# qucontrol/krotov

Hardware: AMD Instinct MI355X
Metric: state*timestep propagations/s (Krotov iterations/s in iterations_per_sec), 256-objective N=64 ensemble (higher is better)
Workload: dtype f64

## Files before the change

krotov_amd/csrc/kh_common.h:

```cpp
#pragma once

#include <hip/hip_runtime.h>
#include <stdint.h>

typedef double2 cplx;

#define KH_TU_ALL 0
#define KH_TU_MAIN 1
#define KH_TU_GENERIC 2
#define KH_TU_MINI 3
#define KH_TU_TILE 4
#define KH_TU_Q2 5
#define KH_TU_STREAM 6
#define KH_TU_ENS 7
#define KH_TU_TILEN 8
#define KH_TU_COOP_STORE 9
#define KH_TU_COOP_UPDATE_A 10
#define KH_TU_COOP_UPDATE_B 11
#define KH_TU_ELL_STORE 12
#define KH_TU_ELL_UPDATE_A 13
#define KH_TU_ELL_UPDATE_B 14
#define KH_TU_TILEX 15
#define KH_TU_LIND 16
#ifndef KH_TU
// ... 70 lines not shown
    int lo = __builtin_amdgcn_readfirstlane(__double2loint(v));
    int hi = __builtin_amdgcn_readfirstlane(__double2hiint(v));
    return __hiloint2double(hi, lo);
}

__device__ __forceinline__ double sum64(double v) {
    v = sum16(v);
    return (readlane_f64(v, 0) + readlane_f64(v, 16)) + (readlane_f64(v, 32) + readlane_f64(v, 48));
}

__device__ __forceinline__ double sum64_mfma(double v) {
    double d = __builtin_amdgcn_mfma_f64_4x4x4f64(v, 1.0, 0.0, 0, 0, 0);
    d += dpp_move<KH_DPP_ROR8>(d);
    d += dpp_move<KH_DPP_ROR4>(d);
    return __builtin_amdgcn_mfma_f64_4x4x4f64(d, 1.0, 0.0, 0, 0, 0);
}

__host__ inline void kh_build_degree_table(double tol, double *tab ) {
    tab[0] = 0.0;
    for (int m = 1; m <= KH_MAX_DEGREE; ++m) {
        double lo = 0.0, hi = (double)(m + 2) * (1.0 - 1e-12);
        for (int it = 0; it < 200; ++it) {
            const double th = 0.5 * (lo + hi);
            double term = 1.0;
            for (int j = 1; j <= m + 1; ++j) term *= th / j;
            if (term <= tol * (1.0 - th / (m + 2))) lo = th; else hi = th;
        }
        tab[m] = lo;
    }
}

#define KH_Q2_ROWS (KH_MAX_DEGREE / 2)

#define KH_RATIO_STRIDE (KH_MAX_DEGREE + 1)

__host__ inline void kh_build_taylor_rows(double *c0 , double *rows ,
                                          double *ratios ) {
    for (int m = 0; m <= KH_MAX_DEGREE; ++m) {
        c0[m] = 1.0;
        ratios[(size_t)m * KH_RATIO_STRIDE] = 1.0;
        for (int j = 1; j <= KH_MAX_DEGREE; ++j) ratios[(size_t)m * KH_RATIO_STRIDE + j] = 1.0 / j;
        for (int p = 0; p < KH_Q2_ROWS; ++p) {
            rows[((size_t)m * KH_Q2_ROWS + p) * 2 + 0] = 1.0 / (2 * p + 1);
            rows[((size_t)m * KH_Q2_ROWS + p) * 2 + 1] = 1.0 / ((2.0 * p + 1) * (2 * p + 2));
        }
    }
}

__host__ inline void kh_bessel_j(double theta, int kmax, long double *J) {
    const int start = kmax + 40 + (int)(2.0 * theta);
    long double jp = 0.0L, jc = 1e-300L, norm = 0.0L;
    for (int k = start; k >= 1; --k) {
        const long double jm = (2.0L * k / (long double)theta) * jc - jp;
        jp = jc;
        jc = jm;
        if (k - 1 <= kmax) J[k - 1] = jc;
        if (((k - 1) & 1) == 0) norm += (k - 1 == 0 ? 1.0L : 2.0L) * jc;
        if (fabsl(jc) > 1e200L) {
            jc *= 1e-200L;
            jp *= 1e-200L;
            norm *= 1e-200L;
            for (int q = k - 1; q <= kmax; ++q) J[q] *= 1e-200L;
        }
    }
    for (int k = 0; k <= kmax; ++k) J[k] /= norm;
}

__host__ inline long double kh_bernstein_eta(long double d) {
    const long double a = sqrtl(fmaxl(0.0L, 1.0L - d * d));
    const long double xr = -2.0L * d * d, xi = 2.0L * a * d;
    const long double r = sqrtl(xr * xr + xi * xi);
    const long double sr = sqrtl(fmaxl(0.0L, 0.5L * (r + xr))), si = sqrtl(fmaxl(0.0L, 0.5L * (r - xr)));
    const long double p = hypotl(a + sr, d + si), q = hypotl(a - sr, d - si);
    return logl(p > q ? p : q);
}
__host__ inline void kh_build_real_spectrum_rows(double tol, double *tab , double *c0, double *rows,
                                                 double *ratios, double theta_cap = 2.0, double delta = 0.0) {
    const int TAIL = 40;
    long double J[KH_MAX_DEGREE + TAIL + 2];
    auto err = [&](double theta, int m) {
        kh_bessel_j(theta, m + TAIL, J);
        long double e = 0.0L;
        if (delta > 0.0) {
            const long double d = (long double)delta / (long double)theta;
            const long double eta = d < 1.0L ? kh_bernstein_eta(d) : 1e3L;
            for (int k = m + 1; k <= m + TAIL; ++k) e += fabsl(J[k]) * coshl(k * eta);
            return (double)(2.0L * (1.0L + sqrtl(2.0L)) * e);
        }
        for (int k = m + 1; k <= m + TAIL; ++k) e += fabsl(J[k]);
        return (double)(2.0L * e);
    };
    kh_build_taylor_rows(c0, rows, ratios);
    double taylor_tab[KH_MAX_DEGREE + 1];
    kh_build_degree_table(tol, taylor_tab);
    tab[0] = 0.0;
    for (int m = 1; m <= KH_MAX_DEGREE; ++m) {
        if (m & 1) {
            tab[m] = tab[m - 1];
            continue;
        }
        if (taylor_tab[m] >= theta_cap) {
            tab[m] = taylor_tab[m] > tab[m - 1] ? taylor_tab[m] : tab[m - 1];
            continue;
        }
        double lo = 0.0, hi = theta_cap;
        if (err(hi, m) <= tol) {
            lo = hi;
        } else {
            for (int it = 0; it < 60; ++it) {
                const double th = 0.5 * (lo + hi);
                if (err(th, m) <= tol) lo = th; else hi = th;
            }
        }
        if (lo < tab[m - 1]) lo = tab[m - 1];
        tab[m] = lo;
        const double theta = lo;
        if (!(theta > 0.0)) continue;
        static long double T[KH_MAX_DEGREE + 1][KH_MAX_DEGREE + 1];
        for (int k = 0; k <= m; ++k)
            for (int j = 0; j <= m; ++j) T[k][j] = 0.0L;
        T[0][0] = 1.0L;
        if (m >= 1) T[1][1] = 1.0L;
        for (int k = 1; k < m; ++k)
            for (int j = 0; j <= k + 1; ++j) T[k + 1][j] = (j > 0 ? 2.0L * T[k][j - 1] : 0.0L) - T[k - 1][j];
        kh_bessel_j(theta, m, J);
        long double c[KH_MAX_DEGREE + 1];
        for (int j = 0; j <= m; ++j) {
            long double acc = 0.0L;
            for (int k = j; k <= m; k += 2)
                acc += (k == 0 ? 1.0L : 2.0L) * J[k] * T[k][j] * (((k - j) / 2) % 2 ? -1.0L : 1.0L);
            c[j] = acc / powl((long double)theta, j);
        }
        c0[m] = (double)c[0];
        ratios[(size_t)m * KH_RATIO_STRIDE] = (double)c[0];
        for (int j = 1; j <= m; ++j) ratios[(size_t)m * KH_RATIO_STRIDE + j] = (double)(j == 1 ? c[1] : c[j] / c[j - 1]);
        for (int p = 0; 2 * p + 2 <= m && p < KH_Q2_ROWS; ++p) {
            const long double den = p == 0 ? 1.0L : c[2 * p];
            rows[((size_t)m * KH_Q2_ROWS + p) * 2 + 0] = (double)(c[2 * p + 1] / den);
            rows[((size_t)m * KH_Q2_ROWS + p) * 2 + 1] = (double)(c[2 * p + 2] / den);
        }
    }
}

struct KhDegreeCache {
    int m;
    double lo, hi;
};

__device__ __forceinline__ void kh_degree_cached(double theta, const double *tab, double theta_max,
                                                 double inv_theta_max, KhDegreeCache &c, int *s_out, int *m_out) {
    int s = 1;
    double th = theta;
    if (theta > theta_max) {
        s = (int)ceil(theta * inv_theta_max);
        th = theta / s;
    }
    if (!(th > c.lo && th <= c.hi)) {
        int m = c.m < 1 ? 1 : c.m;
        while (m > 1 && th <= tab[m - 1]) --m;
        while (m < KH_MAX_DEGREE && th > tab[m]) ++m;
        c.m = m;
        c.lo = m > 1 ? tab[m - 1] : -1.0;
        c.hi = m < KH_MAX_DEGREE ? tab[m] : 1e300;
    }
    *s_out = s;
    *m_out = c.m;
}

__device__ __forceinline__ void kh_degree_lookup(double theta, const double *__restrict__ tab, double theta_max,
                                                 double inv_theta_max, int hint, int *s_out, int *m_out) {
    int s = 1;
    double th = theta;
// ... 262 lines not shown
```

krotov_amd/csrc/kh_coop.h:

```cpp
#pragma once

#include "kh_common.h"
#include "kh_generic.h"

#define KH_COOP_THREADS 512
#define KH_COOP_WAVES 8
#define KH_COOP_COLS 16
#define KH_COOP_RING 32
#ifndef KH_COOP_RING_LOCAL
#define KH_COOP_RING_LOCAL 4
#endif
#ifndef KH_COOP_CHUNK
#define KH_COOP_CHUNK 4
#endif
#define KH_COOP_MAX_L 2

typedef double kh_d4 __attribute__((ext_vector_type(4)));

template <int COLS>
__device__ __forceinline__ bool kh_coop_is_owner(int tid) {
    if constexpr (COLS == 2) return (tid & 15) == 0;
    return tid < 16 * COLS;
}
template <int COLS>
// ... 819 lines not shown
                state.y += t.y;
                if (owner_valid) kh_coop_publish<COLS>(c, rid + 1, y, row, col, j == m ? state : t, c.local != 0);
            }
            ++rid;
        }
    }
    return true;
}

#define KH_COOP_REFRESH 64
struct KhCoopSqMasks {
    unsigned int h0, h1, p0, p1, p2;
};
__device__ __forceinline__ KhCoopSqMasks kh_coop_sq_masks(const KhCoopArgs &c, int g, int wave) {
    KhCoopSqMasks m = {0u, 0u, 0u, 0u, 0u};
    if (c.sq != nullptr) {
        m.h0 = kh_coop_frag_mask(c.tab[0], c.G, g, wave, c.ks);
        m.h1 = kh_coop_frag_mask(c.tab[1], c.G, g, wave, c.ks);
        m.p0 = kh_coop_frag_mask(c.tab[2], c.G, g, wave, c.ks);
        m.p1 = kh_coop_frag_mask(c.tab[3], c.G, g, wave, c.ks);
        m.p2 = kh_coop_frag_mask(c.tab[4], c.G, g, wave, c.ks);
    }
    return m;
}
template <int MAXKS>
__device__ __forceinline__ void kh_coop_sq_restart(const KhCoopArgs &c, const KhCoopSqMasks &mk, int g, int wave,
                                                   int lane, const KhCoopFrag &a, cplx (&breg)[MAXKS],
                                                   double &eps_prev) {
    kh_coop_reg_load<MAXKS>(c.tab[2], g, wave, lane, c.ks, breg, mk.p0);
    kh_coop_load_frag<MAXKS>(c.tab[0], g, wave, lane, c.ks, a, mk.h0);
    eps_prev = 0.0;
}

template <int MAXKS, int COLS>
__device__ __forceinline__ bool kh_coop_expm_action_sq(const KhCoopArgs &c, const KhExchange &ex,
                                                       const KhCoopSqMasks &mk, double eps, double &eps_prev, const KhCoopFrag &a,
                                                       cplx (&breg)[MAXKS],
                                                       cplx &state, unsigned int &rid, KhCoopLds &s, int N, int y,
                                                       int g, int row, int col, bool owner_valid, double fre,
                                                       double fim, double dt, int nsub, int m, int tid, int wave,
                                                       int lane, const cplx (*p1pre)[MAXKS] = nullptr) {
    const double h = kh_uniform(nsub == 1 ? dt : dt / nsub);
    const double f2h2 = kh_uniform((fre * fre - fim * fim) * h * h);
    const int phases = (m + 1) >> 1;
    const bool series = c.ser_rows != nullptr;
    if (series) {
        const double *grow = c.ser_rows + (size_t)m * KH_Q2_ROWS * 2;
        if (tid < 2 * phases) s.coef[tid] = grow[tid];
        if (tid == 2 * phases) s.coef[tid] = c.ser_c0[m];
        __syncthreads();
    }
    const double *rows = series ? s.coef : nullptr;
    const double c_0 = kh_uniform(series ? s.coef[2 * phases] : 1.0), c_1 = kh_uniform(series ? s.coef[0] : 1.0);
#ifndef KH_COOP_X_NOREBUILD
    {
#ifdef KH_TIMING
        const long long tr0 = clock64();
#endif
        const double e1 = eps - eps_prev, e2 = e1 * (eps + eps_prev);
        if (p1pre != nullptr) {
            kh_coop_axpy_pair<MAXKS>(c.tab[4], e2, breg, c.tab[1], e1, a, g, wave, lane, c.ks, mk.p2 | mk.h1);
#pragma unroll
            for (int q = 0; q < MAXKS; ++q) {
                breg[q].x = fma(e1, (*p1pre)[q].x, breg[q].x);
                breg[q].y = fma(e1, (*p1pre)[q].y, breg[q].y);
            }
        } else {
            kh_coop_reg_axpy<MAXKS>(c.tab[3], e1, g, wave, lane, c.ks, breg, mk.p1);
            kh_coop_reg_axpy<MAXKS>(c.tab[4], e2, g, wave, lane, c.ks, breg, mk.p2);
            kh_coop_axpy_frag<MAXKS>(c.tab[1], e1, g, wave, lane, c.ks, a, mk.h1);
        }
        eps_prev = kh_uniform(eps);
#ifdef KH_TIMING
        if (tid == 0 && blockIdx.x == 0) {
            const long long tr1 = clock64();
            s.tim[10] += (double)(tr1 - tr0);
            if (s.tim[11] != 0.0) s.tim[11] += (double)(tr1 - tr0);
        }
#endif
    }
#endif
    const KhCoopRegFrag<MAXKS> bf = {breg, ~0u};
    for (int sub = 0; sub < nsub; ++sub) {
        cplx sacc = c_make(h * c_1 * state.x, h * c_1 * state.y);
        state = c_make(c_0 * state.x, c_0 * state.y);
        for (int ph = 0; ph < phases; ++ph) {
            const double r2 = rows != nullptr ? rows[2 * ph + 1] : kh_inv_table[2 * ph + 1] * kh_inv_table[2 * ph + 2];
            const double r1n = ph + 1 < phases ? (rows != nullptr ? rows[2 * ph + 2] : kh_inv_table[2 * ph + 3]) : 0.0;
            cplx w;
            kh_coop_round<MAXKS, COLS>(c, ex, rid, y, N, bf, s, tid, wave, lane, w);
            const double c2 = f2h2 * r2, hn = h * r1n;
            if (kh_coop_is_owner<COLS>(tid)) {
                const cplx t2 = c_make(c2 * w.x, c2 * w.y);
                state.x += t2.x;
                state.y += t2.y;
                const bool last = (ph + 1 == phases);
                if (!last) {
                    sacc.x = fma(hn, t2.x, sacc.x);
                    sacc.y = fma(hn, t2.y, sacc.y);
                }
                if (owner_valid) kh_coop_publish<COLS>(c, rid + 1, y, row, col, last ? sacc : t2, c.local != 0);
            }
            ++rid;
        }
        cplx w;
        kh_coop_round<MAXKS, COLS>(c, ex, rid, y, N, a, s, tid, wave, lane, w);
        if (s.abort) return false;
        if (kh_coop_is_owner<COLS>(tid)) {
            const cplx odd = c_mul(c_make(fre, fim), w);
            state.x += odd.x;
            state.y += odd.y;
            if (owner_valid) kh_coop_publish<COLS>(c, rid + 1, y, row, col, state, c.local != 0);
        }
        ++rid;
    }
    return true;
}

template <int MAXKS, int COLS>
__device__ __forceinline__ bool kh_coop_expm_action_sq_ahead(const KhCoopArgs &c, const KhExchange &ex, const KhCoopSqMasks &mk,
                                                             double eps, double eps_next, bool have_next, double &eps_b,
                                                             double &eps_a, const KhCoopFrag &a, cplx (&breg)[MAXKS],
                                                             cplx &state, unsigned int &rid, KhCoopLds &s, int N, int y, int g,
                                                             int row, int col, bool owner_valid, double fre, double fim,
                                                             double dt, int nsub, int m, int tid, int wave, int lane) {
    static_assert(MAXKS % 4 == 0, "quarters");
    const double h = kh_uniform(nsub == 1 ? dt : dt / nsub);
    const double f2h2 = kh_uniform((fre * fre - fim * fim) * h * h);
    const int phases = (m + 1) >> 1;
    const bool series = c.ser_rows != nullptr;
    if (series) {
        const double *grow = c.ser_rows + (size_t)m * KH_Q2_ROWS * 2;
        if (tid < 2 * phases) s.coef[tid] = grow[tid];
        if (tid == 2 * phases) s.coef[tid] = c.ser_c0[m];
        __syncthreads();
    }
    const double *rows = series ? s.coef : nullptr;
    const double c_0 = kh_uniform(series ? s.coef[2 * phases] : 1.0), c_1 = kh_uniform(series ? s.coef[0] : 1.0);
    if (eps_b != eps) {
        const double e1 = eps - eps_b, e2 = e1 * (eps + eps_b);
        kh_coop_reg_axpy<MAXKS>(c.tab[3], e1, g, wave, lane, c.ks, breg, mk.p1);
        kh_coop_reg_axpy<MAXKS>(c.tab[4], e2, g, wave, lane, c.ks, breg, mk.p2);
        eps_b = kh_uniform(eps);
    }
    const auto advance_a = [&]() {
        if (eps_a != eps) {
            kh_coop_axpy_frag<MAXKS>(c.tab[1], eps - eps_a, g, wave, lane, c.ks, a, mk.h1);
            eps_a = kh_uniform(eps);
        }
    };
    const KhCoopRegFrag<MAXKS> bf = {breg, ~0u};
    const KhCoopSrc src1 = kh_coop_frag_src(c.tab[3], g, wave, lane, c.ks);
    constexpr int QS = MAXKS / 4;
    for (int sub = 0; sub < nsub; ++sub) {
        const bool ahead = have_next && sub + 1 == nsub;
        const bool staged = ahead && phases >= 4;
        cplx p1n[MAXKS];
#pragma unroll
        for (int q = 0; q < MAXKS; ++q) p1n[q] = c_make(0.0, 0.0);
        cplx sacc = c_make(h * c_1 * state.x, h * c_1 * state.y);
        state = c_make(c_0 * state.x, c_0 * state.y);
        const auto b_round = [&](int ph, const auto &hook2) {
            const double r2 = rows != nullptr ? rows[2 * ph + 1] : kh_inv_table[2 * ph + 1] * kh_inv_table[2 * ph + 2];
            const double r1n = ph + 1 < phases ? (rows != nullptr ? rows[2 * ph + 2] : kh_inv_table[2 * ph + 3]) : 0.0;
            cplx w;
            kh_coop_round<MAXKS, COLS>(c, ex, rid, y, N, bf, s, tid, wave, lane, w, advance_a, hook2);
            const double c2 = f2h2 * r2, hn = h * r1n;
            if (kh_coop_is_owner<COLS>(tid)) {
                const cplx t2 = c_make(c2 * w.x, c2 * w.y);
                state.x += t2.x;
                state.y += t2.y;
                const bool last = (ph + 1 == phases);
                if (!last) {
                    sacc.x = fma(hn, t2.x, sacc.x);
                    sacc.y = fma(hn, t2.y, sacc.y);
                }
                if (owner_valid) kh_coop_publish<COLS>(c, rid + 1, y, row, col, last ? sacc : t2, c.local != 0);
            }
            ++rid;
        };
        const int plain_rounds = staged ? phases - 4 : phases;
        for (int ph = 0; ph < plain_rounds; ++ph) b_round(ph, KhNoHook());
        if (staged) {
            b_round(phases - 4, [&]() {
#pragma unroll
                for (int j = 0; j < QS; ++j) p1n[0 * QS + j] = src1[(size_t)(0 * QS + j) * 64];
            });
            b_round(phases - 3, [&]() {
#pragma unroll
                for (int j = 0; j < QS; ++j) p1n[1 * QS + j] = src1[(size_t)(1 * QS + j) * 64];
            });
            b_round(phases - 2, [&]() {
#pragma unroll
                for (int j = 0; j < QS; ++j) p1n[2 * QS + j] = src1[(size_t)(2 * QS + j) * 64];
            });
            b_round(phases - 1, [&]() {
#pragma unroll
                for (int j = 0; j < QS; ++j) p1n[3 * QS + j] = src1[(size_t)(3 * QS + j) * 64];
            });
        }
        advance_a();
        if (ahead && !staged) kh_coop_reg_load<MAXKS>(c.tab[3], g, wave, lane, c.ks, p1n, mk.p1);
        const auto advance_b = [&]() {
            if (ahead) {
                const double e1 = eps_next - eps_b, e2 = e1 * (eps_next + eps_b);
#pragma unroll
                for (int q = 0; q < MAXKS; ++q) {
                    breg[q].x = fma(e1, p1n[q].x, breg[q].x);
                    breg[q].y = fma(e1, p1n[q].y, breg[q].y);
                }
                kh_coop_reg_axpy<MAXKS>(c.tab[4], e2, g, wave, lane, c.ks, breg, mk.p2);
                eps_b = kh_uniform(eps_next);
            }
        };
        cplx w;
        kh_coop_round<MAXKS, COLS>(c, ex, rid, y, N, a, s, tid, wave, lane, w, advance_b);
        if (s.abort) return false;
        if (kh_coop_is_owner<COLS>(tid)) {
            const cplx odd = c_mul(c_make(fre, fim), w);
            state.x += odd.x;
            state.y += odd.y;
            if (owner_valid) kh_coop_publish<COLS>(c, rid + 1, y, row, col, state, c.local != 0);
        }
        ++rid;
    }
    return true;
}

__global__ void kh_coop_adj_mask_kernel(const cplx *__restrict__ op , int N, int G,
// ... 93 lines not shown
    const KhCoopFrag a = {(cplx *)s.frag + tid};
    cplx breg[MAXKS];
    double eps_prev = 0.0, eps_a = 0.0;
    const KhCoopSqMasks mk = kh_coop_sq_masks(c, g, wave);
#pragma unroll
    for (int q = 0; q < MAXKS; ++q) breg[q] = c_make(0.0, 0.0);
    for (int step = 0; step < nt - 1; ++step) {
        const int n = direction > 0 ? step : nt - 2 - step;
        if (SQ && step % KH_COOP_REFRESH == 0) {
            kh_coop_sq_restart<MAXKS>(c, mk, g, wave, lane, a, breg, eps_prev);
            eps_a = 0.0;
        }
        double eps[KH_COOP_MAX_L];
        double theta = p.op_norms[0];
#pragma unroll
        for (int l = 0; l < KH_COOP_MAX_L; ++l) {
            eps[l] = 0.0;
            if (l < L) {
                eps[l] = pulses[(size_t)l * (nt - 1) + n];
                theta += fabs(eps[l]) * p.op_norms[1 + l];
            }
        }
        const double dt = p.dt[n];
        int nsub, m;
        kh_degree_lookup(theta * dt, s.deg, p.theta_max, p.inv_theta_max, m_hint, &nsub, &m);
        m_hint = m;
        if constexpr (SQ) {
            const bool have_next = step + 1 < nt - 1;
            const double eps_next = have_next ? pulses[direction > 0 ? n + 1 : n - 1] : 0.0;
            if (!kh_coop_expm_action_sq_ahead<MAXKS, COLS>(c, ex, mk, eps[0], eps_next, have_next, eps_prev, eps_a, a, breg, state,
                                                           rid, s, N, y, g, row, col, owner_valid, p.fre, p.fim, dt, nsub, m, tid,
                                                           wave, lane))
                return;
            rounds += (double)nsub * (((m + 1) >> 1) + 1);
        } else {
            kh_coop_build<MAXKS>(c.fops, eps, L, g, wave, lane, c.ks, a);
            if (!kh_coop_expm_action<MAXKS, COLS>(c, ex, a, state, rid, s, N, y, row, col, owner_valid, p.fre, p.fim, dt,
                                                  nsub, m, tid, wave, lane))
                return;
            rounds += (double)nsub * m;
        }
        if (has_state && store != nullptr) store[((size_t)k * nt + (direction > 0 ? n + 1 : n)) * N + row] = state;
    }
    if (has_state && state_out != nullptr) state_out[(size_t)k * N + row] = state;
    if (g == 0 && tid == 0 && p.stats != nullptr) {
        const int cols = min(c.cols, p.K - y * c.cols);
        atomicAdd(p.stats, rounds * cols);
#ifdef KH_TIMING
        if (y == 0) {
            p.stats[1] = s.tim[0] / rounds + 1e6 * (double)(long long)(s.tim[4] / rounds);
            p.stats[2] = s.tim[1] / rounds + 1e6 * (double)(long long)(100.0 * s.tim[5] / rounds);
            p.stats[3] = s.tim[2] / rounds + 1e6 * (double)(long long)(100.0 * s.tim[6] / rounds);
            p.stats[4] = 0.0;
            p.stats[5] = s.tim[0] / rounds;
            p.stats[6] = p.stats[5] + s.tim[1] / rounds;
            p.stats[7] = p.stats[6] + s.tim[2] / rounds;
            p.stats[8] = p.stats[7] + s.tim[7] / rounds;
            p.stats[9] = p.stats[8] + s.tim[8] / rounds;
            p.stats[10] = p.stats[9] + s.tim[9] / rounds;
            p.stats[11] = s.tim[10] / (nt - 1);
            p.stats[12] = 1.0 + s.local;
            p.stats[13] = 0.0;
        }
#endif
    }
}

// ... 125 lines not shown
            }
#ifdef KH_TIMING
            if (g == 0 && lane == 0 && p.stats != nullptr && y < 16) p.stats[20 + y] += (double)(clock64() - tx0) / (nt - 1);
#endif
#endif
            if (lane == 0) {
#pragma unroll
                for (int l = 0; l < KH_COOP_MAX_L; ++l) s.D[par][l] = D[l];
                s.D[par][KH_COOP_MAX_L] = ok ? 1.0 : 0.0;
            }
        }
        __syncthreads();
        if (s.D[par][KH_COOP_MAX_L] == 0.0) return;
        const double dt = kh_uniform(p.dt[n]);
        double eps[KH_COOP_MAX_L];
        double theta = kh_uniform(p.op_norms[0]);
#pragma unroll
        for (int l = 0; l < KH_COOP_MAX_L; ++l) {
            if (l >= L) break;
            const double d1 = kh_uniform(s.D[par][l]);
            const double stepw = kh_uniform(u.shape[(size_t)l * (nt - 1) + n] / u.lambda[l]);
            eps[l] = kh_uniform(u.guess[(size_t)l * (nt - 1) + n] + stepw * d1);
            g_a_loc[l] = kh_uniform(g_a_loc[l] + stepw * (d1 * d1) * dt);
            theta = kh_uniform(theta + fabs(eps[l]) * p.op_norms[1 + l]);
            if (wg == 0 && tid == 0) u.opt[(size_t)l * (nt - 1) + n] = eps[l];
        }
        int nsub, m;
        kh_degree_lookup(theta * dt, s.deg, p.theta_max, p.inv_theta_max, m_hint, &nsub, &m);
        m_hint = m;
        if constexpr (ADJ) {
            if (!kh_coop_expm_action_sq<MAXKS, COLS>(c, ex, mk, eps[0], eps_prev, a, breg, state, rid, s, N, y, g, row, col,
                                                     owner_valid, p.fre, p.fim, dt, nsub, m, tid, wave, lane, &p1pre))
                return;
            rounds += nsub * (((m + 1) >> 1) + 1);
        } else if constexpr (SQ) {
            if (!kh_coop_expm_action_sq<MAXKS, COLS>(c, ex, mk, eps[0], eps_prev, a, breg, state, rid, s, N, y, g, row, col,
                                                     owner_valid, p.fre, p.fim, dt, nsub, m, tid, wave, lane))
                return;
            rounds += nsub * (((m + 1) >> 1) + 1);
        } else {
            kh_coop_build<MAXKS>(c.fops, eps, L, g, wave, lane, c.ks, a);
            if (!kh_coop_expm_action<MAXKS, COLS>(c, ex, a, state, rid, s, N, y, row, col, owner_valid, p.fre, p.fim, dt,
                                                  nsub, m, tid, wave, lane))
                return;
            rounds += nsub * m;
        }
    }
    if (has_state) {
        u.phi[(size_t)k * N + row] = state;
        if constexpr (SO) u.fw_store[((size_t)k * nt + (nt - 1)) * N + row] = state;
    }
    if (wg == 0 && tid == 0) {
#pragma unroll
        for (int l = 0; l < KH_COOP_MAX_L; ++l)
            if (l < L) u.g_a[l] = g_a_loc[l];
    }
#ifdef KH_TIMING
    if (blockIdx.x == 0 && tid == 0 && p.stats != nullptr) {
        p.stats[28] = s.tim[10] / (nt - 1);
        p.stats[29] = (s.tim[0] + s.tim[1] + s.tim[2] + s.tim[7] + s.tim[8]) / (nt - 1);
        p.stats[30] = s.tim[9] / (nt - 1);
    }
#endif
    if (g == 0 && tid == 0 && p.stats != nullptr) {
        const int cols = min(c.cols, p.K - y * c.cols);
        atomicAdd(p.stats, (double)rounds * cols);
    }
}
```

krotov_amd/csrc/kh_ens.h:

```cpp
#pragma once
#include "kh_tile64.h"

#define KH_ENS_THREADS 512
#define KH_ENS_WAVES 8
#define KH_ENS_MAXCG 8

struct KhEnsArgs {
    const cplx *H0;
    const cplx *H1;
    const double *scale;
};

__host__ __device__ constexpr int kh_ens_np(int ncg) { return ncg == 1 ? 1 : ncg / 2; }
__host__ __device__ constexpr int kh_ens_w(int ncg) { return ncg == 1 ? 1 : 2; }
__host__ __device__ constexpr int kh_ens_buf(int ncg) { return 512 * ncg; }
__host__ inline size_t kh_ens_lds_bytes(int ncg) { return (size_t)2 * kh_ens_buf(ncg) * sizeof(double); }
__host__ inline size_t kh_ens2_lds_bytes(int ncg) {
    return ((size_t)3 * kh_ens_buf(ncg) + (size_t)KH_ENS_WAVES * 32 * 64) * sizeof(double);
}

__global__ void __launch_bounds__(256)
kh_ens_detect_kernel(const cplx *const *ops, int K, int N, int ref_idx, int ref_comp, double *scale, int *flags)
#if KH_DEFINES(KH_TU_MAIN)
{
// ... 464 lines not shown
        if (w == 0 && tid == 0) u.opt[n] = eps;
        int nsub, m;
        kh_degree_lookup((n0 + fabs(eps) * n1) * dt, deg_sh, p.theta_max, p.inv_theta_max, m_loaded < 1 ? 12 : m_loaded, &nsub, &m);
        if (m != m_loaded) {
            __syncthreads();
            if (tid < KH_Q2_ROWS) {
                const double *rr = p.q2_rows + ((size_t)m * KH_Q2_ROWS + tid) * 2;
                rows_sh[tid] = make_double2(rr[0], rr[1]);
            }
            if (tid == KH_Q2_ROWS) rows_sh[KH_Q2_ROWS] = make_double2(p.q2_c0[m], 0.0);
            __syncthreads();
        }
        m_loaded = m;
        const double h = nsub == 1 ? dt : dt / nsub;
        const double f2h2 = f2 * h * h;
        const int phases = (m + 1) >> 1;
        for (int sub = 0; sub < nsub; ++sub) {
            if (sub > 0) {
                pass3(xf + cur * BUF + lane_off, zA, zB);
                matvecs += 3.0 * n_valid;
            }
            const double hr0 = h * rows_sh[0].x, c0 = rows_sh[KH_Q2_ROWS].x;
            double sacc[NCG];
#pragma unroll
            for (int cg = 0; cg < NCG; ++cg) {
                sacc[cg] = hr0 * S[cg];
                S[cg] *= c0;
            }
            if (phases == 1) {
                write_x(xs, sacc);
                __syncthreads();
            }
            for (int ph = 0; ph < phases; ++ph) {
                if (ph > 0) {
                    pass3(xf + cur * BUF + lane_off, zA, zB);
                    matvecs += 3.0 * n_valid;
                }
                const double c2 = f2h2 * rows_sh[ph].y;
                const bool last = ph + 1 == phases;
                double t2[NCG];
#pragma unroll
                for (int cg = 0; cg < NCG; ++cg) {
                    const double se = es[cg] * eps;
                    const double z1 = dpp_move<KH_DPP_ROR8>(zA[cg]);
                    const double z2 = zB[cg] + dpp_move<KH_DPP_ROR8>(zB[cg]);
                    t2[cg] = c2 * fma(se, fma(se, z2, z1), zA[cg]);
                    S[cg] += t2[cg];
                }
                if (!last) {
                    const double hn = h * rows_sh[ph + 1].x;
#pragma unroll
                    for (int cg = 0; cg < NCG; ++cg) sacc[cg] = fma(hn, t2[cg], sacc[cg]);
                    write_x(xf + (cur ^ 1) * BUF, t2);
                    if (ph + 2 == phases) write_x(xs, sacc);
                } else {
                    double yC[NCG];
                    double afC[32];
#pragma unroll
                    for (int ks = 0; ks < 32; ++ks) afC[ks] = afc_lds[ks * 64];
                    pass(xs + lane_off, afC, yC);
                    matvecs += 2.0 * n_valid;
#pragma unroll
                    for (int cg = 0; cg < NCG; ++cg) {
                        const double a = fma(es[cg] * eps, dpp_move<KH_DPP_ROR8>(yC[cg]), yC[cg]);
                        const double other = dpp_move<KH_DPP_XOR1>(a);
                        S[cg] += fma(cis_sign * p.fim, other, p.fre * a);
                    }
                    write_x(xf + (cur ^ 1) * BUF, S);
                    if (sub + 1 == nsub && n + 1 < nt - 1) sums((n + 1) & 1);
                }
                __syncthreads();
                cur ^= 1;
            }
        }
    }
    if (owner && r < N) {
#pragma unroll
        for (int cg = 0; cg < NCG; ++cg) {
            const int k = w * CPW + 2 * cg + (q >> 1);
            if (k < K) ((double *)u.phi)[((size_t)k * N + r) * 2 + pc] = S[cg];
// ... 6 lines not shown
```

krotov_amd/csrc/kh_mini.h:

```cpp
#pragma once

#include "kh_common.h"
#include "kh_generic.h"

#define KH_MINI_N 16
#define KH_MINI_MAXK 8

struct KhMiniLds {
    double2 rows[KH_MAX_DEGREE + 1][KH_Q2_ROWS];
    double c0[KH_MAX_DEGREE + 1];
    double deg[KH_MAX_DEGREE + 1];
    double part[2][KH_MINI_MAXK];
    double D[2][2];
};

__device__ __forceinline__ void kh_mini_stage_tables(const KhSweepArgs &p, KhMiniLds &s, int tid, int nthreads) {
    for (int i = tid; i < (KH_MAX_DEGREE + 1) * KH_Q2_ROWS; i += nthreads) {
        s.rows[i / KH_Q2_ROWS][i % KH_Q2_ROWS] = make_double2(p.q2_rows[2 * (size_t)i], p.q2_rows[2 * (size_t)i + 1]);
    }
    for (int i = tid; i <= KH_MAX_DEGREE; i += nthreads) {
        s.c0[i] = p.q2_c0[i];
        s.deg[i] = p.q2_theta[i];
    }
}
// ... 18 lines not shown
    return c_make(sum4(y.x), sum4(y.y));
}

#define KH_MINI_PHASES 8
struct KhMiniCoef {
    int m, nsub;
    double dt;
    double c0, hr;
    double c2[KH_MINI_PHASES];
    double hn[KH_MINI_PHASES];
};

__device__ __forceinline__ void kh_mini_coefficients(KhMiniCoef &c, const KhMiniLds &s, int m, int nsub, double dt,
                                                     double fre, double fim) {
    if (c.m == m && c.nsub == nsub && c.dt == dt) return;
    c.m = m;
    c.nsub = nsub;
    c.dt = dt;
    const double h = nsub == 1 ? dt : dt / nsub;
    const double f2h2 = (fre * fre - fim * fim) * h * h;
    const double2 *rows = s.rows[m];
    c.c0 = s.c0[m];
    c.hr = h * rows[0].x;
#pragma unroll
    for (int q = 0; q < KH_MINI_PHASES; ++q) {
        c.c2[q] = f2h2 * rows[q].y;
        c.hn[q] = h * rows[q + 1].x;
    }
}

__device__ __forceinline__ int kh_mini_expm_action(const cplx (&a)[4], const cplx (&b)[4], cplx &state,
                                                   const KhMiniLds &s, const KhMiniCoef &c, double fre, double fim,
                                                   double dt, int nsub, int m, int lane) {
    const int phases = (m + 1) >> 1;
    for (int sub = 0; sub < nsub; ++sub) {
        cplx term = state;
        cplx sacc = c_make(c.hr * state.x, c.hr * state.y);
        state = c_make(c.c0 * state.x, c.c0 * state.y);
        if (phases <= KH_MINI_PHASES) {
#pragma unroll
            for (int ph = 0; ph < KH_MINI_PHASES; ++ph) {
                if (ph < phases) {
                    const cplx yb = kh_mini_matvec(b, term, lane);
                    term = c_make(c.c2[ph] * yb.x, c.c2[ph] * yb.y);
                    state.x += term.x;
                    state.y += term.y;
                    if (ph + 1 < phases) {
                        sacc.x = fma(c.hn[ph], term.x, sacc.x);
                        sacc.y = fma(c.hn[ph], term.y, sacc.y);
                    }
                }
            }
        } else {
            const double h = nsub == 1 ? dt : dt / nsub;
            const double f2h2 = (fre * fre - fim * fim) * h * h;
            const double2 *rows = s.rows[m];
            for (int ph = 0; ph < phases; ++ph) {
                const double c2 = f2h2 * rows[ph].y;
                const cplx yb = kh_mini_matvec(b, term, lane);
                term = c_make(c2 * yb.x, c2 * yb.y);
                state.x += term.x;
                state.y += term.y;
                if (ph + 1 < phases) {
                    const double hn = h * rows[ph + 1].x;
                    sacc.x = fma(hn, term.x, sacc.x);
                    sacc.y = fma(hn, term.y, sacc.y);
                }
            }
        }
        const cplx odd = c_mul(c_make(fre, fim), kh_mini_matvec(a, sacc, lane));
        state.x += odd.x;
        state.y += odd.y;
    }
    return nsub * (phases + 1);
}

__device__ __forceinline__ void kh_mini_build(double eps, const cplx (&h0)[4], const cplx (&h1)[4], const cplx (&p0)[4],
                                              const cplx (&p1)[4], const cplx (&p2)[4], cplx (&a)[4], cplx (&b)[4]) {
    const double eps2 = eps * eps;
#pragma unroll
    for (int j = 0; j < 4; ++j) {
        a[j] = c_make(fma(eps, h1[j].x, h0[j].x), fma(eps, h1[j].y, h0[j].y));
        b[j] = c_make(fma(eps2, p2[j].x, fma(eps, p1[j].x, p0[j].x)), fma(eps2, p2[j].y, fma(eps, p1[j].y, p0[j].y)));
    }
}

__global__ void __launch_bounds__(64)
kh_mini_sweep_store(KhSweepArgs p, const cplx *const *__restrict__ sq, const double *__restrict__ pulses,
                    const cplx *__restrict__ state_in, cplx *__restrict__ store, cplx *__restrict__ state_out,
                    int direction)
#if KH_DEFINES(KH_TU_MINI)
{
    __shared__ KhMiniLds s;
    const int lane = threadIdx.x, r = lane >> 2, k = blockIdx.x;
    const bool writer = (lane & 3) == 0;
    const int N = p.N, nt = p.nt;
    kh_mini_stage_tables(p, s, lane, 64);
    cplx h0[4], h1[4], p0[4], p1[4], p2[4];
    kh_mini_load_tile(p.ops[(size_t)k * 2], N, lane, h0);
    kh_mini_load_tile(p.ops[(size_t)k * 2 + 1], N, lane, h1);
    kh_mini_load_tile(sq[(size_t)k * 3], N, lane, p0);
    kh_mini_load_tile(sq[(size_t)k * 3 + 1], N, lane, p1);
    kh_mini_load_tile(sq[(size_t)k * 3 + 2], N, lane, p2);
    const double nrm0 = p.op_norms[(size_t)k * 2], nrm1 = p.op_norms[(size_t)k * 2 + 1];
    cplx state = r < N ? state_in[(size_t)k * N + r] : c_make(0.0, 0.0);
    __syncthreads();
    const bool stores = store != nullptr && writer && r < N;
// ... 122 lines not shown
        int nsub, m;
        kh_degree_cached((nrm0 + fabs(eps) * nrm1) * dt, s.deg, p.theta_max, p.inv_theta_max, dc, &nsub, &m);
        kh_mini_coefficients(coef, s, m, nsub, dt, p.fre, p.fim);
        cplx a[4], b[4];
        kh_mini_build(eps, h0, h1, p0, p1, p2, a, b);
        matvecs += kh_mini_expm_action(a, b, state, s, coef, p.fre, p.fim, dt, nsub, m, lane);
        if (n + 1 < nt - 1) partial(n + 1);
        __syncthreads();
    }
    if (writer && r < N) {
        u.phi[(size_t)k * N + r] = state;
        if constexpr (SO) u.fw_store[((size_t)k * nt + u.n_end) * N + r] = state;
    }
    if (tid == 0) u.g_a[0] = g_a_loc;
    if (lane == 0 && p.stats != nullptr) atomicAdd(p.stats, matvecs);
}

#define KH_QUAD_N 4
#define KH_QUAD_MAXK 4

__device__ __forceinline__ cplx kh_quad_load(const cplx *op, int N, int r, int c, bool valid) {
    return (valid && op != nullptr && r < N && c < N) ? op[(size_t)r * N + c] : c_make(0.0, 0.0);
}

__device__ __forceinline__ cplx kh_quad_matvec(cplx t, cplx v, int lane) {
    const int src = (lane & 48) | ((lane & 3) << 2);
    const cplx x = c_make(__shfl(v.x, src), __shfl(v.y, src));
    const cplx y = c_mul(t, x);
    return c_make(sum4(y.x), sum4(y.y));
}

__device__ __forceinline__ int kh_quad_expm_action(cplx a, cplx b, cplx &state, const KhMiniLds &s, const KhMiniCoef &c,
                                                   double fre, double fim, double dt, int nsub, int m, int lane) {
    const int phases = (m + 1) >> 1;
    for (int sub = 0; sub < nsub; ++sub) {
        cplx term = state;
        cplx sacc = c_make(c.hr * state.x, c.hr * state.y);
        state = c_make(c.c0 * state.x, c.c0 * state.y);
        if (phases <= KH_MINI_PHASES) {
#pragma unroll
            for (int ph = 0; ph < KH_MINI_PHASES; ++ph) {
                if (ph < phases) {
                    const cplx yb = kh_quad_matvec(b, term, lane);
                    term = c_make(c.c2[ph] * yb.x, c.c2[ph] * yb.y);
                    state.x += term.x;
                    state.y += term.y;
                    if (ph + 1 < phases) {
                        sacc.x = fma(c.hn[ph], term.x, sacc.x);
                        sacc.y = fma(c.hn[ph], term.y, sacc.y);
                    }
                }
            }
        } else {
            const double h = nsub == 1 ? dt : dt / nsub;
            const double f2h2 = (fre * fre - fim * fim) * h * h;
            const double2 *rows = s.rows[m];
            for (int ph = 0; ph < phases; ++ph) {
                const double c2 = f2h2 * rows[ph].y;
                const cplx yb = kh_quad_matvec(b, term, lane);
                term = c_make(c2 * yb.x, c2 * yb.y);
                state.x += term.x;
                state.y += term.y;
                if (ph + 1 < phases) {
                    const double hn = h * rows[ph + 1].x;
                    sacc.x = fma(hn, term.x, sacc.x);
                    sacc.y = fma(hn, term.y, sacc.y);
                }
            }
        }
        const cplx odd = c_mul(c_make(fre, fim), kh_quad_matvec(a, sacc, lane));
        state.x += odd.x;
        state.y += odd.y;
    }
    return nsub * (phases + 1);
}

__device__ __forceinline__ double kh_wave_max(double v) {
#pragma unroll
    for (int off = 1; off < 64; off <<= 1) v = fmax(v, __shfl_xor(v, off));
    return v;
}

struct KhQuadTiles {
    cplx h0, h1, p0, p1, p2;
    double nrm0, nrm1;
};

__device__ __forceinline__ KhQuadTiles kh_quad_load_tiles(const KhSweepArgs &p, const cplx *const *sq, int k, int r, int c,
                                                          bool valid) {
    KhQuadTiles t;
    const size_t kk = valid ? (size_t)k : 0;
    t.h0 = kh_quad_load(p.ops[kk * 2], p.N, r, c, valid);
    t.h1 = kh_quad_load(p.ops[kk * 2 + 1], p.N, r, c, valid);
    t.p0 = kh_quad_load(sq[kk * 3], p.N, r, c, valid);
    t.p1 = kh_quad_load(sq[kk * 3 + 1], p.N, r, c, valid);
    t.p2 = kh_quad_load(sq[kk * 3 + 2], p.N, r, c, valid);
    t.nrm0 = valid ? p.op_norms[kk * 2] : 0.0;
    t.nrm1 = valid ? p.op_norms[kk * 2 + 1] : 0.0;
    return t;
}

__device__ __forceinline__ void kh_quad_build(const KhQuadTiles &t, double eps, cplx &a, cplx &b) {
    const double eps2 = eps * eps;
    a = c_make(fma(eps, t.h1.x, t.h0.x), fma(eps, t.h1.y, t.h0.y));
    b = c_make(fma(eps2, t.p2.x, fma(eps, t.p1.x, t.p0.x)), fma(eps2, t.p2.y, fma(eps, t.p1.y, t.p0.y)));
}

// ... 139 lines not shown
```

krotov_amd/csrc/kh_tile64q2.h:

```cpp
#pragma once

#include "kh_common.h"
#include "kh_generic.h"
#include "kh_tile64.h"

#define KH_Q2_THREADS 512
#ifdef KH_Q2_DPP_REDUCE
typedef KhLanes<false> KhQ2Lanes;
#else
typedef KhLanes<true> KhQ2Lanes;
#endif
#define KH_Q2_TILE_ELEMS (8 * KH_Q2_THREADS)

struct KhQ2Lds {
    cplx *h0;
    cplx *p0;
    cplx (*buf)[KH_TILE_N];
    cplx *chib;
    cplx *sbuf;
    double *red;
    double *D;
    double2 *inv2;
    double *deg;
};
// ... 72 lines not shown
    for (int j = 0; j < 8; ++j) {
        a[j].x = fma(e1, h1[j].x, a[j].x);
        a[j].y = fma(e1, h1[j].y, a[j].y);
        b[j].x = fma(e2, p2[j].x, fma(e1, p1[j].x, b[j].x));
        b[j].y = fma(e2, p2[j].y, fma(e1, p1[j].y, b[j].y));
    }
}

__device__ __forceinline__ void kh_q2_advance(const KhQ2Lds &s, int tid, double eps, double eps_prev, const cplx (&h1)[8],
                                              cplx (&a)[8], cplx (&b)[8]) {
    const double e1 = eps - eps_prev, e2 = e1 * (eps + eps_prev);
#pragma unroll
    for (int j = 0; j < 8; ++j) {
        const cplx q1 = s.h0[j * KH_Q2_THREADS + tid];
        const cplx q2 = s.p0[j * KH_Q2_THREADS + tid];
        a[j].x = fma(e1, h1[j].x, a[j].x);
        a[j].y = fma(e1, h1[j].y, a[j].y);
        b[j].x = fma(e2, q2.x, fma(e1, q1.x, b[j].x));
        b[j].y = fma(e2, q2.y, fma(e1, q1.y, b[j].y));
    }
}

template <class Epilogue>
__device__ __forceinline__ int kh_q2_expm_action(const cplx (&a)[8], const cplx (&b)[8], cplx &state,
                                                 cplx (*buf)[KH_TILE_N], cplx *sbuf, const double2 *inv2, int &cur,
                                                 cplx *store_in, int N, double fre, double fim,
                                                 double dt, int nsub, int m, int wave, int lane,
                                                 Epilogue epilogue) {
    const int cg = KhQ2Lanes::cg(lane), row = wave * 8 + KhQ2Lanes::row_out(lane);
    const bool writer = (lane & 7) == 0;
    const double h = nsub == 1 ? dt : dt / nsub;
    const double f2h2 = (fre * fre - fim * fim) * h * h;
    const int phases = (m + 1) >> 1;
    if (store_in != nullptr && wave == 0 && lane < N) {
        store_in[lane] = buf[cur][lane];
    }
    for (int sub = 0; sub < nsub; ++sub) {
        const double hr = h * inv2[0].x, c0 = inv2[KH_Q2_ROWS].x;
        cplx sacc = c_make(hr * state.x, hr * state.y);
        state = c_make(c0 * state.x, c0 * state.y);
        if (phases == 1) {
            if (writer) sbuf[row] = sacc;
            __syncthreads();
        }
        for (int ph = 0; ph < phases; ++ph) {
            const double c2 = f2h2 * inv2[ph].y;
            cplx xv[8];
#pragma unroll
            for (int j = 0; j < 8; ++j) xv[j] = buf[cur][cg + 8 * j];
            const bool last = (ph + 1 == phases);
            cplx yb = c_make(0.0, 0.0);
#pragma unroll
            for (int j = 0; j < 8; ++j) c_fma(yb, b[j], xv[j]);
            const double t2x = KhQ2Lanes::rowsum(yb.x, c2), t2y = KhQ2Lanes::rowsum(yb.y, c2);
            state.x += t2x;
            state.y += t2y;
            if (!last) {
                const double hn = h * inv2[ph + 1].x;
                sacc.x = fma(hn, t2x, sacc.x);
                sacc.y = fma(hn, t2y, sacc.y);
                if (writer) {
                    buf[cur ^ 1][row] = c_make(t2x, t2y);
                    if (ph + 2 == phases) sbuf[row] = sacc;
                }
            } else {
                __builtin_amdgcn_sched_barrier(0);
                cplx sv[8];
#pragma unroll
                for (int j = 0; j < 8; ++j) sv[j] = sbuf[cg + 8 * j];
                cplx ya = c_make(0.0, 0.0);
#pragma unroll
                for (int j = 0; j < 8; ++j) c_fma(ya, a[j], sv[j]);
                const cplx odd = c_mul(c_make(fre, fim), c_make(KhQ2Lanes::rowsum(ya.x, 1.0), KhQ2Lanes::rowsum(ya.y, 1.0)));
                state.x += odd.x;
                state.y += odd.y;
                if (writer) buf[cur ^ 1][row] = c_make(state.x, state.y);
                if (sub + 1 == nsub) epilogue();
            }
            __syncthreads();
            cur ^= 1;
        }
    }
    return nsub * (phases + 1);
}

__global__ void __launch_bounds__(KH_Q2_THREADS)
kh_q2_sweep_store(KhSweepArgs p, const cplx *const *__restrict__ sq, const double *__restrict__ pulses,
                  const cplx *__restrict__ state_in, cplx *__restrict__ store, cplx *__restrict__ state_out,
                  int direction)
#if KH_DEFINES(KH_TU_Q2)
{
    extern __shared__ __attribute__((aligned(16))) char smem[];
    const KhQ2Lds s = kh_q2_carve(smem);
    const int tid = threadIdx.x, wave = tid >> 6, lane = tid & 63;
    if (tid <= KH_MAX_DEGREE) s.deg[tid] = p.q2_theta[tid];
    const int row = wave * 8 + KhQ2Lanes::row_out(lane);
    const bool writer = (lane & 7) == 0;
    const int N = p.N, nt = p.nt;
    double matvecs = 0.0;
    for (int k = blockIdx.x; k < p.K; k += gridDim.x) {
        const cplx *const *ops_k = p.ops + (size_t)k * 2;
        const cplx *const *sq_k = sq + (size_t)k * 3;
        __syncthreads();
        kh_q2_stage_tile(ops_k[0], N, wave, lane, tid, s.h0);
        kh_q2_stage_tile(sq_k[0], N, wave, lane, tid, s.p0);
        cplx h1[8], p1[8], p2[8];
        kh_q2_load_tile(ops_k[1], N, wave, lane, h1);
        kh_q2_load_tile(sq_k[1], N, wave, lane, p1);
        kh_q2_load_tile(sq_k[2], N, wave, lane, p2);
        const double nrm0 = p.op_norms[(size_t)k * 2], nrm1 = p.op_norms[(size_t)k * 2 + 1];

        cplx state = row < N ? state_in[(size_t)k * N + row] : c_make(0.0, 0.0);
        int cur = 0;
        if (writer) s.buf[0][row] = state;
        __syncthreads();
        const int n0 = direction > 0 ? 0 : nt - 2;
// ... 329 lines not shown
```

Baseline: 65.99 million.

## Allow odd series degrees and skip the trailing even B-product

Odd polynomial degrees become usable in the degree table, which previously rounded them up to the next even degree. The coefficient rows for odd m now get a zeroed final even term. Each expm-action variant (coop, ensemble, mini/quad, tile q2) runs only m/2 B matvec rounds and skips the last even product when m is odd. The aim is to save about one matrix-vector product per substep when an odd degree meets the tolerance. In exchange it changes degree selection and error bounds and adds branches in the phase loops.

```diff
diff --git a/krotov_amd/csrc/kh_common.h b/krotov_amd/csrc/kh_common.h
--- a/krotov_amd/csrc/kh_common.h
+++ b/krotov_amd/csrc/kh_common.h
@@ -126,6 +126,8 @@
 
 #define KH_Q2_ROWS (KH_MAX_DEGREE / 2)
 
+__host__ __device__ __forceinline__ int kh_series_b_products(int m) { return m >> 1; }
+
 #define KH_RATIO_STRIDE (KH_MAX_DEGREE + 1)
 
 __host__ inline void kh_build_taylor_rows(double *c0 , double *rows ,
@@ -138,6 +140,7 @@
             rows[((size_t)m * KH_Q2_ROWS + p) * 2 + 0] = 1.0 / (2 * p + 1);
             rows[((size_t)m * KH_Q2_ROWS + p) * 2 + 1] = 1.0 / ((2.0 * p + 1) * (2 * p + 2));
         }
+        if (m & 1) rows[((size_t)m * KH_Q2_ROWS + (m >> 1)) * 2 + 1] = 0.0;
     }
 }
 
@@ -189,10 +192,6 @@
     kh_build_degree_table(tol, taylor_tab);
     tab[0] = 0.0;
     for (int m = 1; m <= KH_MAX_DEGREE; ++m) {
-        if (m & 1) {
-            tab[m] = tab[m - 1];
-            continue;
-        }
         if (taylor_tab[m] >= theta_cap) {
             tab[m] = taylor_tab[m] > tab[m - 1] ? taylor_tab[m] : tab[m - 1];
             continue;
@@ -228,10 +227,10 @@
         c0[m] = (double)c[0];
         ratios[(size_t)m * KH_RATIO_STRIDE] = (double)c[0];
         for (int j = 1; j <= m; ++j) ratios[(size_t)m * KH_RATIO_STRIDE + j] = (double)(j == 1 ? c[1] : c[j] / c[j - 1]);
-        for (int p = 0; 2 * p + 2 <= m && p < KH_Q2_ROWS; ++p) {
+        for (int p = 0; 2 * p + 1 <= m && p < KH_Q2_ROWS; ++p) {
             const long double den = p == 0 ? 1.0L : c[2 * p];
             rows[((size_t)m * KH_Q2_ROWS + p) * 2 + 0] = (double)(c[2 * p + 1] / den);
-            rows[((size_t)m * KH_Q2_ROWS + p) * 2 + 1] = (double)(c[2 * p + 2] / den);
+            rows[((size_t)m * KH_Q2_ROWS + p) * 2 + 1] = 2 * p + 2 <= m ? (double)(c[2 * p + 2] / den) : 0.0;
         }
     }
 }
diff --git a/krotov_amd/csrc/kh_coop.h b/krotov_amd/csrc/kh_coop.h
--- a/krotov_amd/csrc/kh_coop.h
+++ b/krotov_amd/csrc/kh_coop.h
@@ -875,6 +875,8 @@
     eps_prev = 0.0;
 }
 
+__host__ __device__ __forceinline__ int kh_coop_sq_b_rounds(int m) { return m > 1 ? kh_series_b_products(m) : 1; }
+
 template <int MAXKS, int COLS>
 __device__ __forceinline__ bool kh_coop_expm_action_sq(const KhCoopArgs &c, const KhExchange &ex,
                                                        const KhCoopSqMasks &mk, double eps, double &eps_prev, const KhCoopFrag &a,
@@ -885,7 +887,7 @@
                                                        int lane, const cplx (*p1pre)[MAXKS] = nullptr) {
     const double h = kh_uniform(nsub == 1 ? dt : dt / nsub);
     const double f2h2 = kh_uniform((fre * fre - fim * fim) * h * h);
-    const int phases = (m + 1) >> 1;
+    const int phases = (m + 1) >> 1, nb = kh_coop_sq_b_rounds(m);
     const bool series = c.ser_rows != nullptr;
     if (series) {
         const double *grow = c.ser_rows + (size_t)m * KH_Q2_ROWS * 2;
@@ -927,7 +929,7 @@
     for (int sub = 0; sub < nsub; ++sub) {
         cplx sacc = c_make(h * c_1 * state.x, h * c_1 * state.y);
         state = c_make(c_0 * state.x, c_0 * state.y);
-        for (int ph = 0; ph < phases; ++ph) {
+        for (int ph = 0; ph < nb; ++ph) {
             const double r2 = rows != nullptr ? rows[2 * ph + 1] : kh_inv_table[2 * ph + 1] * kh_inv_table[2 * ph + 2];
             const double r1n = ph + 1 < phases ? (rows != nullptr ? rows[2 * ph + 2] : kh_inv_table[2 * ph + 3]) : 0.0;
             cplx w;
@@ -937,8 +939,8 @@
                 const cplx t2 = c_make(c2 * w.x, c2 * w.y);
                 state.x += t2.x;
                 state.y += t2.y;
-                const bool last = (ph + 1 == phases);
-                if (!last) {
+                const bool last = (ph + 1 == nb);
+                if (ph + 1 < phases) {
                     sacc.x = fma(hn, t2.x, sacc.x);
                     sacc.y = fma(hn, t2.y, sacc.y);
                 }
@@ -970,7 +972,7 @@
     static_assert(MAXKS % 4 == 0, "quarters");
     const double h = kh_uniform(nsub == 1 ? dt : dt / nsub);
     const double f2h2 = kh_uniform((fre * fre - fim * fim) * h * h);
-    const int phases = (m + 1) >> 1;
+    const int phases = (m + 1) >> 1, nb = kh_coop_sq_b_rounds(m);
     const bool series = c.ser_rows != nullptr;
     if (series) {
         const double *grow = c.ser_rows + (size_t)m * KH_Q2_ROWS * 2;
@@ -997,7 +999,7 @@
     constexpr int QS = MAXKS / 4;
     for (int sub = 0; sub < nsub; ++sub) {
         const bool ahead = have_next && sub + 1 == nsub;
-        const bool staged = ahead && phases >= 4;
+        const bool staged = ahead && nb >= 4;
         cplx p1n[MAXKS];
 #pragma unroll
         for (int q = 0; q < MAXKS; ++q) p1n[q] = c_make(0.0, 0.0);
@@ -1013,8 +1015,8 @@
                 const cplx t2 = c_make(c2 * w.x, c2 * w.y);
                 state.x += t2.x;
                 state.y += t2.y;
-                const bool last = (ph + 1 == phases);
-                if (!last) {
+                const bool last = (ph + 1 == nb);
+                if (ph + 1 < phases) {
                     sacc.x = fma(hn, t2.x, sacc.x);
                     sacc.y = fma(hn, t2.y, sacc.y);
                 }
@@ -1022,22 +1024,22 @@
             }
             ++rid;
         };
-        const int plain_rounds = staged ? phases - 4 : phases;
+        const int plain_rounds = staged ? nb - 4 : nb;
         for (int ph = 0; ph < plain_rounds; ++ph) b_round(ph, KhNoHook());
         if (staged) {
-            b_round(phases - 4, [&]() {
+            b_round(nb - 4, [&]() {
 #pragma unroll
                 for (int j = 0; j < QS; ++j) p1n[0 * QS + j] = src1[(size_t)(0 * QS + j) * 64];
             });
-            b_round(phases - 3, [&]() {
+            b_round(nb - 3, [&]() {
 #pragma unroll
                 for (int j = 0; j < QS; ++j) p1n[1 * QS + j] = src1[(size_t)(1 * QS + j) * 64];
             });
-            b_round(phases - 2, [&]() {
+            b_round(nb - 2, [&]() {
 #pragma unroll
                 for (int j = 0; j < QS; ++j) p1n[2 * QS + j] = src1[(size_t)(2 * QS + j) * 64];
             });
-            b_round(phases - 1, [&]() {
+            b_round(nb - 1, [&]() {
 #pragma unroll
                 for (int j = 0; j < QS; ++j) p1n[3 * QS + j] = src1[(size_t)(3 * QS + j) * 64];
             });
@@ -1197,7 +1199,7 @@
                                                            rid, s, N, y, g, row, col, owner_valid, p.fre, p.fim, dt, nsub, m, tid,
                                                            wave, lane))
                 return;
-            rounds += (double)nsub * (((m + 1) >> 1) + 1);
+            rounds += (double)nsub * (kh_coop_sq_b_rounds(m) + 1);
         } else {
             kh_coop_build<MAXKS>(c.fops, eps, L, g, wave, lane, c.ks, a);
             if (!kh_coop_expm_action<MAXKS, COLS>(c, ex, a, state, rid, s, N, y, row, col, owner_valid, p.fre, p.fim, dt,
@@ -1389,12 +1391,12 @@
             if (!kh_coop_expm_action_sq<MAXKS, COLS>(c, ex, mk, eps[0], eps_prev, a, breg, state, rid, s, N, y, g, row, col,
                                                      owner_valid, p.fre, p.fim, dt, nsub, m, tid, wave, lane, &p1pre))
                 return;
-            rounds += nsub * (((m + 1) >> 1) + 1);
+            rounds += nsub * (kh_coop_sq_b_rounds(m) + 1);
         } else if constexpr (SQ) {
             if (!kh_coop_expm_action_sq<MAXKS, COLS>(c, ex, mk, eps[0], eps_prev, a, breg, state, rid, s, N, y, g, row, col,
                                                      owner_valid, p.fre, p.fim, dt, nsub, m, tid, wave, lane))
                 return;
-            rounds += nsub * (((m + 1) >> 1) + 1);
+            rounds += nsub * (kh_coop_sq_b_rounds(m) + 1);
         } else {
             kh_coop_build<MAXKS>(c.fops, eps, L, g, wave, lane, c.ks, a);
             if (!kh_coop_expm_action<MAXKS, COLS>(c, ex, a, state, rid, s, N, y, row, col, owner_valid, p.fre, p.fim, dt,
diff --git a/krotov_amd/csrc/kh_ens.h b/krotov_amd/csrc/kh_ens.h
--- a/krotov_amd/csrc/kh_ens.h
+++ b/krotov_amd/csrc/kh_ens.h
@@ -520,20 +520,25 @@
                 __syncthreads();
             }
             for (int ph = 0; ph < phases; ++ph) {
-                if (ph > 0) {
+                const bool last = ph + 1 == phases;
+                const bool even_pass = !(last && (m & 1));
+                if (ph > 0 && even_pass) {
                     pass3(xf + cur * BUF + lane_off, zA, zB);
                     matvecs += 3.0 * n_valid;
                 }
-                const double c2 = f2h2 * rows_sh[ph].y;
-                const bool last = ph + 1 == phases;
                 double t2[NCG];
 #pragma unroll
-                for (int cg = 0; cg < NCG; ++cg) {
-                    const double se = es[cg] * eps;
-                    const double z1 = dpp_move<KH_DPP_ROR8>(zA[cg]);
-                    const double z2 = zB[cg] + dpp_move<KH_DPP_ROR8>(zB[cg]);
-                    t2[cg] = c2 * fma(se, fma(se, z2, z1), zA[cg]);
-                    S[cg] += t2[cg];
+                for (int cg = 0; cg < NCG; ++cg) t2[cg] = 0.0;
+                if (even_pass) {
+                    const double c2 = f2h2 * rows_sh[ph].y;
+#pragma unroll
+                    for (int cg = 0; cg < NCG; ++cg) {
+                        const double se = es[cg] * eps;
+                        const double z1 = dpp_move<KH_DPP_ROR8>(zA[cg]);
+                        const double z2 = zB[cg] + dpp_move<KH_DPP_ROR8>(zB[cg]);
+                        t2[cg] = c2 * fma(se, fma(se, z2, z1), zA[cg]);
+                        S[cg] += t2[cg];
+                    }
                 }
                 if (!last) {
                     const double hn = h * rows_sh[ph + 1].x;
diff --git a/krotov_amd/csrc/kh_mini.h b/krotov_amd/csrc/kh_mini.h
--- a/krotov_amd/csrc/kh_mini.h
+++ b/krotov_amd/csrc/kh_mini.h
@@ -74,7 +74,7 @@
 __device__ __forceinline__ int kh_mini_expm_action(const cplx (&a)[4], const cplx (&b)[4], cplx &state,
                                                    const KhMiniLds &s, const KhMiniCoef &c, double fre, double fim,
                                                    double dt, int nsub, int m, int lane) {
-    const int phases = (m + 1) >> 1;
+    const int phases = (m + 1) >> 1, nb = kh_series_b_products(m);
     for (int sub = 0; sub < nsub; ++sub) {
         cplx term = state;
         cplx sacc = c_make(c.hr * state.x, c.hr * state.y);
@@ -82,7 +82,7 @@
         if (phases <= KH_MINI_PHASES) {
 #pragma unroll
             for (int ph = 0; ph < KH_MINI_PHASES; ++ph) {
-                if (ph < phases) {
+                if (ph < nb) {
                     const cplx yb = kh_mini_matvec(b, term, lane);
                     term = c_make(c.c2[ph] * yb.x, c.c2[ph] * yb.y);
                     state.x += term.x;
@@ -97,7 +97,7 @@
             const double h = nsub == 1 ? dt : dt / nsub;
             const double f2h2 = (fre * fre - fim * fim) * h * h;
             const double2 *rows = s.rows[m];
-            for (int ph = 0; ph < phases; ++ph) {
+            for (int ph = 0; ph < nb; ++ph) {
                 const double c2 = f2h2 * rows[ph].y;
                 const cplx yb = kh_mini_matvec(b, term, lane);
                 term = c_make(c2 * yb.x, c2 * yb.y);
@@ -114,7 +114,7 @@
         state.x += odd.x;
         state.y += odd.y;
     }
-    return nsub * (phases + 1);
+    return nsub * (nb + 1);
 }
 
 __device__ __forceinline__ void kh_mini_build(double eps, const cplx (&h0)[4], const cplx (&h1)[4], const cplx (&p0)[4],
@@ -303,7 +303,7 @@
 
 __device__ __forceinline__ int kh_quad_expm_action(cplx a, cplx b, cplx &state, const KhMiniLds &s, const KhMiniCoef &c,
                                                    double fre, double fim, double dt, int nsub, int m, int lane) {
-    const int phases = (m + 1) >> 1;
+    const int phases = (m + 1) >> 1, nb = kh_series_b_products(m);
     for (int sub = 0; sub < nsub; ++sub) {
         cplx term = state;
         cplx sacc = c_make(c.hr * state.x, c.hr * state.y);
@@ -311,7 +311,7 @@
         if (phases <= KH_MINI_PHASES) {
 #pragma unroll
             for (int ph = 0; ph < KH_MINI_PHASES; ++ph) {
-                if (ph < phases) {
+                if (ph < nb) {
                     const cplx yb = kh_quad_matvec(b, term, lane);
                     term = c_make(c.c2[ph] * yb.x, c.c2[ph] * yb.y);
                     state.x += term.x;
@@ -326,7 +326,7 @@
             const double h = nsub == 1 ? dt : dt / nsub;
             const double f2h2 = (fre * fre - fim * fim) * h * h;
             const double2 *rows = s.rows[m];
-            for (int ph = 0; ph < phases; ++ph) {
+            for (int ph = 0; ph < nb; ++ph) {
                 const double c2 = f2h2 * rows[ph].y;
                 const cplx yb = kh_quad_matvec(b, term, lane);
                 term = c_make(c2 * yb.x, c2 * yb.y);
@@ -343,7 +343,7 @@
         state.x += odd.x;
         state.y += odd.y;
     }
-    return nsub * (phases + 1);
+    return nsub * (nb + 1);
 }
 
 __device__ __forceinline__ double kh_wave_max(double v) {
diff --git a/krotov_amd/csrc/kh_tile64q2.h b/krotov_amd/csrc/kh_tile64q2.h
--- a/krotov_amd/csrc/kh_tile64q2.h
+++ b/krotov_amd/csrc/kh_tile64q2.h
@@ -128,6 +128,7 @@
     const double h = nsub == 1 ? dt : dt / nsub;
     const double f2h2 = (fre * fre - fim * fim) * h * h;
     const int phases = (m + 1) >> 1;
+    const bool odd_m = (m & 1) != 0;
     if (store_in != nullptr && wave == 0 && lane < N) {
         store_in[lane] = buf[cur][lane];
     }
@@ -140,17 +141,21 @@
             __syncthreads();
         }
         for (int ph = 0; ph < phases; ++ph) {
-            const double c2 = f2h2 * inv2[ph].y;
-            cplx xv[8];
-#pragma unroll
-            for (int j = 0; j < 8; ++j) xv[j] = buf[cur][cg + 8 * j];
             const bool last = (ph + 1 == phases);
-            cplx yb = c_make(0.0, 0.0);
-#pragma unroll
-            for (int j = 0; j < 8; ++j) c_fma(yb, b[j], xv[j]);
-            const double t2x = KhQ2Lanes::rowsum(yb.x, c2), t2y = KhQ2Lanes::rowsum(yb.y, c2);
-            state.x += t2x;
-            state.y += t2y;
+            double t2x = 0.0, t2y = 0.0;
+            if (!(last && odd_m)) {
+                const double c2 = f2h2 * inv2[ph].y;
+                cplx xv[8];
+#pragma unroll
+                for (int j = 0; j < 8; ++j) xv[j] = buf[cur][cg + 8 * j];
+                cplx yb = c_make(0.0, 0.0);
+#pragma unroll
+                for (int j = 0; j < 8; ++j) c_fma(yb, b[j], xv[j]);
+                t2x = KhQ2Lanes::rowsum(yb.x, c2);
+                t2y = KhQ2Lanes::rowsum(yb.y, c2);
+                state.x += t2x;
+                state.y += t2y;
+            }
             if (!last) {
                 const double hn = h * inv2[ph + 1].x;
                 sacc.x = fma(hn, t2x, sacc.x);
@@ -177,7 +182,7 @@
             cur ^= 1;
         }
     }
-    return nsub * (phases + 1);
+    return nsub * (kh_series_b_products(m) + 1);
 }
 
 __global__ void __launch_bounds__(KH_Q2_THREADS)
```

After: 66.42 million, median of 5. No clear change (+0.7%).
